# Leqr/MSMP-PDE

Measured on AMD Instinct MI355X. Metric: rollout-steps/sec (whole node), E2 nx=100 tw=25, higher is better.
Workload: dtype f32; 1 GPU; E2 MSMP-PDE (MP_PDE_SolverLEMLinGated), 2048 graphs x nx=100, time_window=25, 6 gated layer pairs, radius graph n=3; graphs_total=2048, graphs_per_gpu=2048, nodes_per_gpu=204800, edges_per_gpu=1204224, parallelism=dp1 (graph-sharded, no collective in the rollout), sub_batches=1, range_policy_switched_to_exact_fp32=False, preheat=163 untimed steps (>= 1 s) after the 5 warm-up steps

## Files before the change

### msmp-pde_amd/csrc/mlp_kernels.hip

```cpp
#include "mfma_tiles.h"

namespace msmp {

struct EdgeArgs {
    const float* h;
    const float* u;
    const float* pos;
    const float* vars;
    const int* tgt;
    const int* col;
    const int* rowptr;
    long n_edges, n_nodes;
    int tile_nodes;
    int xcd_map;
    int tw, nv, nc1;
    const float* w1;
    const float* w2;
    const float* w2s;
    const float* scales;
    const float* b1;
    const float* b2;
    const float* P;
    const float* Q;
    float* msg;
// ... 730 lines not shown
        const f32x4 v0 = *reinterpret_cast<const f32x4*>(row32 + 16 * s + 8 * hh);
        const f32x4 v1 = *reinterpret_cast<const f32x4*>(row32 + 16 * s + 8 * hh + 4);
        const float v[8] = {v0[0], v0[1], v0[2], v0[3], v1[0], v1[1], v1[2], v1[3]};
        split8(v, bhi[0][s], blo[0][s]);
    }
}

struct NodeSplitArgs {
    NodeArgs b;
    const float* w3s;
    const float* scales;
};

__device__ __forceinline__ void node_head_split(const float* __restrict__ h, const float* __restrict__ agg, const float* __restrict__ vars,
                                                long nc, int nv, const float* b3, const float* b4, const float* w3v, const float* w3s,
                                                const float* scales, float* lds, int tid, int lane, int hh, f32x16 (&y)[4][1]) {
    const float sc3 = scales[2], inv3 = scales[6], sc4 = scales[3], inv4 = scales[7];
    f32x16 z[4][1];
    acc_init_bias<1>(b3, hh, z);
    for (int v = 0; v < nv; ++v) {
        const float xv = vars[(size_t)nc * nv + v];
#pragma unroll
        for (int T = 0; T < 4; ++T)
#pragma unroll
            for (int r = 0; r < 16; ++r)
                z[T][0][r] = fmaf(w3v[(32 * T + acc_row(r, hh)) * MSMP_MAX_VARS + v], xv, z[T][0][r]);
    }
#pragma unroll
    for (int T = 0; T < 4; ++T)
#pragma unroll
        for (int r = 0; r < 16; ++r) z[T][0][r] *= sc3;

    f32x4 pf[4][4];
    auto row_load = [&](int ch, f32x4 (&dst)[4]) {
        const float* row32 = (ch < 4 ? h : agg) + (size_t)nc * H + 32 * (ch & 3);
#pragma unroll
        for (int s = 0; s < 2; ++s) {
            dst[2 * s] = *reinterpret_cast<const f32x4*>(row32 + 16 * s + 8 * hh);
            dst[2 * s + 1] = *reinterpret_cast<const f32x4*>(row32 + 16 * s + 8 * hh + 4);
        }
    };
#pragma unroll
    for (int ch = 0; ch < 4; ++ch) row_load(ch, pf[ch]);
    WStage ws;
    wstage_load(ws, w3s, tid);
    wstage_store_linear(ws, lds, tid);
    __syncthreads();
#pragma unroll
    for (int ch = 0; ch < 8; ++ch) {
        wstage_load(ws, w3s + (size_t)(ch + 1) * SPLIT_CHUNK_FLOATS, tid);
        half8 bhi[1][2], blo[1][2];
#pragma unroll
        for (int s = 0; s < 2; ++s) {
            const f32x4 v0 = pf[ch & 3][2 * s], v1 = pf[ch & 3][2 * s + 1];
            const float v[8] = {v0[0], v0[1], v0[2], v0[3], v1[0], v1[1], v1[2], v1[3]};
            split8(v, bhi[0][s], blo[0][s]);
        }
        if (ch + 4 < 8) row_load(ch + 4, pf[ch & 3]);
        mma_chunk_split<1>(lds + (ch & 1) * SPLIT_CHUNK_FLOATS, lane, bhi, blo, z);
        wstage_store_linear(ws, lds + ((ch + 1) & 1) * SPLIT_CHUNK_FLOATS, tid);
        __syncthreads();
    }
#pragma unroll
    for (int T = 0; T < 4; ++T)
#pragma unroll
        for (int r = 0; r < 16; ++r) z[T][0][r] = swishf(z[T][0][r] * inv3);

    acc_init_bias_scaled<1>(b4, sc4, hh, y);
    const float* w4s = w3s + 8 * SPLIT_CHUNK_FLOATS;
#pragma unroll
    for (int t = 0; t < 4; ++t) {
        if (t < 3) wstage_load(ws, w4s + (size_t)(t + 1) * SPLIT_CHUNK_FLOATS, tid);
        half8 bhi[1][2], blo[1][2];
        split_acc_tile<1>(z[t], bhi, blo);
        mma_chunk_split<1>(lds + (t & 1) * SPLIT_CHUNK_FLOATS, lane, bhi, blo, y);
        if (t < 3) {
            wstage_store_linear(ws, lds + ((t + 1) & 1) * SPLIT_CHUNK_FLOATS, tid);
            __syncthreads();
        }
    }
#pragma unroll
    for (int T = 0; T < 4; ++T)
#pragma unroll
        for (int r = 0; r < 16; ++r) y[T][0][r] *= inv4;
}

__global__ __launch_bounds__(256, 2) void node_update_split_kernel(NodeSplitArgs sa) {
    __shared__ __attribute__((aligned(16))) float lds[2 * SPLIT_CHUNK_FLOATS];
    const NodeArgs& a = sa.b;
    const int tid = threadIdx.x, lane = tid & 63, wave = tid >> 6;
    const int c = lane & 31, hh = lane >> 5;
    const long n = (long)blockIdx.x * 128 + wave * 32 + c;
    const long nc = n < a.n_nodes ? n : a.n_nodes - 1;
    f32x16 y[4][1];
    node_head_split(a.h, a.agg, a.vars, nc, a.nv, a.b3, a.b4, a.w3v, sa.w3s, sa.scales, lds, tid, lane, hh, y);
    if (n < a.n_nodes) {
        float* o = a.out + (size_t)n * H + 4 * hh;
        const float* hx = a.h + (size_t)n * H + 4 * hh;
#pragma unroll
        for (int T = 0; T < 4; ++T)
#pragma unroll
            for (int q = 0; q < 4; ++q) {
                f32x4 v;
                if (a.mode == MSMP_LAYER_LIN) {
#pragma unroll
                    for (int m = 0; m < 4; ++m) v[m] = y[T][0][4 * q + m];
                } else {
                    const f32x4 x = *reinterpret_cast<const f32x4*>(hx + 32 * T + 8 * q);
#pragma unroll
                    for (int m = 0; m < 4; ++m) v[m] = x[m] + swishf(y[T][0][4 * q + m]);
                }
                *reinterpret_cast<f32x4*>(o + 32 * T + 8 * q) = v;
            }
    }
}

struct TailArgs {
    const float* h;
    const float* agg[2];
    const float* vars;
    const int* graph_ptr;
    int nv, mode;
    float eps;
    const float* b3[2];
    const float* b4[2];
    const float* w3vh[2];
    const float* w3s[2];
    const float* w4t[2];
    const float* scales[2];
    float* out;
    int* status;
};

constexpr float TAIL_ACT_SCALE = 64.0f;
constexpr float TAIL_NODE_SCALE = 256.0f;
__device__ __forceinline__ float tail_node_scaled(float x) { return __builtin_amdgcn_fmed3f(x * TAIL_NODE_SCALE, -65504.0f, 65504.0f); }

constexpr int ROWBUF_FLOATS = 128 * 32;
__device__ __forceinline__ void tail_rows_issue(const float* __restrict__ h, const float* __restrict__ agg, int n0, int n1, int ch, float* buf, int tid) {
    const float* src = (ch < 4 ? h : agg) + 32 * (ch & 3);
#pragma unroll
    for (int i = 0; i < 4; ++i) {
        const int P = tid + 256 * i, r = P >> 3;
        const int node = min(n0 + r, n1 - 1);
        const float* g = src + (size_t)node * H + 4 * ((P & 7) ^ ((r >> 1) & 7));
        __builtin_amdgcn_global_load_lds((const __attribute__((address_space(1))) void*)g, (__attribute__((address_space(3))) void*)(buf + 4 * P), 16, 0, 0);
    }
}
__device__ __forceinline__ void tail_rows_read(const float* buf, int row, int hh, f32x4 (&dst)[4]) {
    const float* rb = buf + row * 32;
    const int sw = (row >> 1) & 7;
#pragma unroll
    for (int s = 0; s < 2; ++s) {
        dst[2 * s] = *reinterpret_cast<const f32x4*>(rb + 4 * ((4 * s + 2 * hh) ^ sw));
        dst[2 * s + 1] = *reinterpret_cast<const f32x4*>(rb + 4 * ((4 * s + 2 * hh + 1) ^ sw));
    }
}

__device__ __forceinline__ void wstage_dma(const float* __restrict__ chunk, float* buf, int tid) {
#pragma unroll
    for (int i = 0; i < 4; ++i)
        __builtin_amdgcn_global_load_lds((const __attribute__((address_space(1))) void*)(chunk + 4 * (tid + 256 * i)),
                                         (__attribute__((address_space(3))) void*)(buf + 4 * (tid + 256 * i)), 16, 0, 0);
}

__device__ __forceinline__ void tail_bias_load(const float* b3, int hh, f32x16 (&z)[4][1]) {
#pragma unroll
    for (int T = 0; T < 4; ++T)
#pragma unroll
        for (int q = 0; q < 4; ++q) {
            const f32x4 bv = *reinterpret_cast<const f32x4*>(b3 + 32 * T + 8 * q + 4 * hh);
#pragma unroll
            for (int m = 0; m < 4; ++m) z[T][0][4 * q + m] = bv[m];
        }
}
__device__ __forceinline__ void tail_bias_pin(f32x16 (&z)[4][1]) {
#pragma unroll
    for (int T = 0; T < 4; ++T) asm volatile("" : "+v"(z[T][0]));
}
__device__ __forceinline__ void tail_bias_scale(f32x16 (&z)[4][1], float sc3) {
#pragma unroll
    for (int T = 0; T < 4; ++T)
#pragma unroll
        for (int r = 0; r < 16; ++r) z[T][0][r] *= sc3;
}
__device__ __forceinline__ float tail_sc3(const float* scales) { return uniform_ro(scales, 2) * TAIL_NODE_SCALE; }

__device__ __forceinline__ void tail_chunk_frags(const float* buf, int myrow, int hh, half8 (&bhi)[1][2], half8 (&blo)[1][2]) {
    f32x4 pf[4];
    tail_rows_read(buf, myrow, hh, pf);
#pragma unroll
    for (int s = 0; s < 2; ++s) {
        const f32x4 v0 = pf[2 * s], v1 = pf[2 * s + 1];
        const float v[8] = {v0[0], v0[1], v0[2], v0[3], v1[0], v1[1], v1[2], v1[3]};
        split8_node(v, bhi[0][s], blo[0][s]);
    }
}

template <int CH0, int PB>
__device__ __forceinline__ void head_chunks(float* rowbuf, int n0, int n1, const float* __restrict__ h, const float* __restrict__ agg, const float* w3vh,
                                            const float* w3s, const float* w4t, float* lds, int tid, int lane, int myrow, int hh, f32x16 (&z)[4][1],
                                            half8 (&wvf)[2][4] PROF_ARGS) {
#pragma unroll
    for (int ch = CH0; ch < 8; ++ch) {
        if (ch < 7) tail_rows_issue(h, agg, n0, n1, ch + 1, rowbuf + ((ch + 1) & 1) * ROWBUF_FLOATS, tid);
        wstage_dma(ch < 7 ? w3s + (size_t)(ch + 1) * SPLIT_CHUNK_FLOATS : w4t, lds + ((ch + 1) & 1) * SPLIT_CHUNK_FLOATS, tid);
        half8 bhi[1][2], blo[1][2];
        tail_chunk_frags(rowbuf + (ch & 1) * ROWBUF_FLOATS, myrow, hh, bhi, blo);
        if (ch == 5) {
            const half8* wv = reinterpret_cast<const half8*>(w3vh) + lane;
#pragma unroll
            for (int m = 0; m < 2; ++m)
#pragma unroll
                for (int T = 0; T < 4; ++T) wvf[m][T] = wv[(m * 4 + T) * 64];
        }
        PROF_MARK(PB);
        mma_chunk_split<1>(lds + (ch & 1) * SPLIT_CHUNK_FLOATS, lane, bhi, blo, z);
        PROF_MARK(PB + 1);
        __syncthreads();
        PROF_MARK(PB + 2);
    }
}

__device__ __forceinline__ void tail_var_frags(const float* xvl, int myrow, int hh, half8 (&bx)[2]) {
    const f32x4 x0 = *reinterpret_cast<const f32x4*>(xvl + 8 * myrow), x1 = *reinterpret_cast<const f32x4*>(xvl + 8 * myrow + 4);
    const float xr[8] = {x0[0], x0[1], x0[2], x0[3], x1[0], x1[1], x1[2], x1[3]};
    float xv[8];
#pragma unroll
    for (int f = 0; f < 8; ++f) xv[f] = tail_node_scaled(xr[f]);
    var_slot_frags(xv, hh, bx);
}

template <typename MidHook, typename LastHook>
__device__ __forceinline__ void head_finish(const float* b4, const float* w4t, const float* scales, float* lds, int tid, int lane, int c, int hh,
                                            f32x16 (&z)[4][1], const half8 (&wvf)[2][4], const half8 (&bx)[2], f32x16 (&yT)[4], MidHook mid_hook,
                                            LastHook last_hook, bool center, float* zref) {
    const float inv3 = uniform_ro(scales, 6) * (TAIL_ACT_SCALE / TAIL_NODE_SCALE), sc4 = uniform_ro(scales, 3) * TAIL_ACT_SCALE;
#pragma unroll
    for (int m = 0; m < 2; ++m)
#pragma unroll
        for (int T = 0; T < 4; ++T) z[T][0] = __builtin_amdgcn_mfma_f32_32x32x16_f16(wvf[m][T], bx[m], z[T][0], 0, 0, 0);
    mid_hook();
    __builtin_amdgcn_sched_barrier(0);
#pragma unroll
    for (int T = 0; T < 4; ++T)
#pragma unroll
        for (int r = 0; r < 16; ++r) {
#if MSMP_PRECISE_ACT
            z[T][0][r] = TAIL_ACT_SCALE * swishf(z[T][0][r] * inv3 * (1.0f / TAIL_ACT_SCALE));
#else
            const float xs = z[T][0][r] * inv3;
            const float e = __builtin_amdgcn_exp2f(xs * (-1.44269504088896340736f / TAIL_ACT_SCALE));
            z[T][0][r] = xs * __builtin_amdgcn_rcpf(1.0f + e);
#endif
        }

    if (center) {
        if ((tid >> 6) == 0 && c == 0) {
#pragma unroll
            for (int T = 0; T < 4; ++T)
#pragma unroll
                for (int q = 0; q < 4; ++q)
                    *reinterpret_cast<f32x4*>(zref + 32 * T + 8 * q + 4 * hh) = f32x4{z[T][0][4 * q], z[T][0][4 * q + 1], z[T][0][4 * q + 2], z[T][0][4 * q + 3]};
        }
        __syncthreads();
#pragma unroll
        for (int T = 0; T < 4; ++T)
#pragma unroll
            for (int q = 0; q < 4; ++q) {
                const f32x4 rv = *reinterpret_cast<const f32x4*>(zref + 32 * T + 8 * q + 4 * hh);
#pragma unroll
                for (int m = 0; m < 4; ++m) z[T][0][4 * q + m] -= rv[m];
            }
    }
    {
        const f32x4 bv = center ? f32x4{0.f, 0.f, 0.f, 0.f} : *reinterpret_cast<const f32x4*>(b4 + 4 * c) * sc4;
#pragma unroll
        for (int T = 0; T < 4; ++T)
#pragma unroll
            for (int r = 0; r < 16; ++r) yT[T][r] = bv[T];
    }
#pragma unroll
    for (int t = 0; t < 4; ++t) {
        if (t < 3) wstage_dma(w4t + (size_t)(t + 1) * SPLIT_CHUNK_FLOATS, lds + ((t + 1) & 1) * SPLIT_CHUNK_FLOATS, tid);
        else last_hook();
        __builtin_amdgcn_sched_barrier(0);
        half8 zhi[1][2], zlo[1][2];
        split_acc_tile<1>(z[t], zhi, zlo);
        const half8* w = reinterpret_cast<const half8*>(lds + (t & 1) * SPLIT_CHUNK_FLOATS) + lane;
#pragma unroll
        for (int s = 0; s < 2; ++s)
#pragma unroll
            for (int T = 0; T < 4; ++T) {
                const half8 whi = w[((s * 4 + T) * 2 + 0) * 64], wlo = w[((s * 4 + T) * 2 + 1) * 64];
                MSMP_MFMA_LOLO(1, yT[T], zlo[0][s], wlo);
                yT[T] = __builtin_amdgcn_mfma_f32_32x32x16_f16(zhi[0][s], wlo, yT[T], 0, 0, 0);
                yT[T] = __builtin_amdgcn_mfma_f32_32x32x16_f16(zlo[0][s], whi, yT[T], 0, 0, 0);
                yT[T] = __builtin_amdgcn_mfma_f32_32x32x16_f16(zhi[0][s], whi, yT[T], 0, 0, 0);
            }
        if (t < 3) __syncthreads();
    }
}

__device__ __forceinline__ void tile_t_total(const float (&v)[4], float* part, float* tot, int tid, int wave, int c, int hh,
                                             float (&out)[4]) {
#pragma unroll
    for (int T = 0; T < 4; ++T) part[(wave * 2 + hh) * H + 32 * T + c] = v[T];
    __syncthreads();
    if (tid < H) {
        float s = 0.f;
#pragma unroll
        for (int p = 0; p < 8; ++p) s += part[p * H + tid];
        tot[tid] = s;
    }
    __syncthreads();
#pragma unroll
    for (int T = 0; T < 4; ++T) out[T] = tot[32 * T + c];
}

__device__ __forceinline__ void tile_t_instance_norm(f32x16 (&x)[4], int wave, int cnt, float unit, float eps, float* part, float* tot,
                                                     int tid, int c, int hh, int* status) {
    const float inv = 1.0f / (float)max(cnt, 1);
    const bool ragged = wave * 32 + 32 > cnt;
    if (ragged) {
#pragma unroll
        for (int T = 0; T < 4; ++T)
#pragma unroll
            for (int r = 0; r < 16; ++r) x[T][r] = wave * 32 + acc_row(r, hh) < cnt ? x[T][r] : 0.f;
    }
    float s[4], m[4];
#pragma unroll
    for (int T = 0; T < 4; ++T) {
        float a0 = 0.f, a1 = 0.f;
#pragma unroll
        for (int r = 0; r < 16; r += 2) { a0 += x[T][r]; a1 += x[T][r + 1]; }
        s[T] = a0 + a1;
    }
    tile_t_total(s, part, tot, tid, wave, c, hh, m);
#pragma unroll
    for (int T = 0; T < 4; ++T) {
        const float mean = m[T] * inv;
        float a0 = 0.f, a1 = 0.f;
#pragma unroll
        for (int r = 0; r < 16; r += 2) {
            x[T][r] -= mean;
            x[T][r + 1] -= mean;
            if (ragged) {
                x[T][r] = wave * 32 + acc_row(r, hh) < cnt ? x[T][r] : 0.f;
                x[T][r + 1] = wave * 32 + acc_row(r + 1, hh) < cnt ? x[T][r + 1] : 0.f;
            }
            a0 = fmaf(x[T][r], x[T][r], a0);
            a1 = fmaf(x[T][r + 1], x[T][r + 1], a1);
        }
        s[T] = a0 + a1;
    }
    tile_t_total(s, part, tot, tid, wave, c, hh, m);
    if (wave == 0 && !(m[0] + m[1] + m[2] + m[3] < 3.0e38f)) status_raise(status, MSMP_STATUS_NONFINITE);
#pragma unroll
    for (int T = 0; T < 4; ++T) {
        const float f = unit * msmp_rsq(m[T] * inv * unit * unit + eps);
#pragma unroll
        for (int r = 0; r < 16; ++r) x[T][r] *= f;
    }
}

template <bool GATED>
__global__ __launch_bounds__(256, 2) void node_tail_split_kernel(TailArgs a) {
    __shared__ __attribute__((aligned(16))) float smem[2 * SPLIT_CHUNK_FLOATS + 2 * ROWBUF_FLOATS + 9 * H + 8 * 128];
    float* const lds = smem;
    float* const rowbuf = smem + 2 * SPLIT_CHUNK_FLOATS;
    float* const part = rowbuf + 2 * ROWBUF_FLOATS;
    float* const tot = part + 8 * H;
    float* const xvl = tot + H;
    const int tid = threadIdx.x, lane = tid & 63, wave = tid >> 6;
    const int c = lane & 31, hh = lane >> 5;
    const int n0 = a.graph_ptr[blockIdx.x], n1 = a.graph_ptr[blockIdx.x + 1];
    const int cnt = n1 - n0;
    if (cnt <= 0) return;

    PROF_DECL
#pragma unroll
    for (int i = 0; i < 4; ++i) {
        const int e = tid + 256 * i, row = e >> 3, f = e & 7;
        const float v = a.vars[(size_t)min(n0 + row, n1 - 1) * a.nv + min(f, a.nv - 1)];
        xvl[e] = v * (row < cnt && f < a.nv ? 1.0f : 0.f);
    }
    const int myrow = wave * 32 + c;
    f32x16 tau[4], y[4];
    f32x16 z[4][1];
    half8 wvf[2][4], bx[2];
    if (GATED) {
        f32x16 zg[4][1];
        tail_rows_issue(a.h, a.agg[1], n0, n1, 0, rowbuf, tid);
        wstage_dma(a.w3s[1], lds, tid);
        tail_bias_load(a.b3[1], hh, zg);
        tail_bias_load(a.b3[0], hh, z);
        tail_bias_pin(zg);
        tail_bias_pin(z);
        tail_bias_scale(zg, tail_sc3(a.scales[1]));
        tail_bias_scale(z, tail_sc3(a.scales[0]));
        __syncthreads();
        PROF_MARK(5);
        half8 bhi[1][2], blo[1][2];
#pragma unroll
        for (int s = 0; s < 8; ++s) {
            const int ch = s >> 1;
            if (!(s & 1)) {
                tail_rows_issue(a.h, a.agg[1], n0, n1, ch + 1, rowbuf + ((ch + 1) & 1) * ROWBUF_FLOATS, tid);
                wstage_dma(a.w3s[0] + (size_t)ch * SPLIT_CHUNK_FLOATS, lds + SPLIT_CHUNK_FLOATS, tid);
                __builtin_amdgcn_sched_barrier(0);
                tail_chunk_frags(rowbuf + (ch & 1) * ROWBUF_FLOATS, myrow, hh, bhi, blo);
                PROF_MARK(6);
                mma_chunk_split<1>(lds, lane, bhi, blo, zg);
            } else {
                wstage_dma(a.w3s[1] + (size_t)(ch + 1) * SPLIT_CHUNK_FLOATS, lds, tid);
                __builtin_amdgcn_sched_barrier(0);
                PROF_MARK(6);
                mma_chunk_split<1>(lds + SPLIT_CHUNK_FLOATS, lane, bhi, blo, z);
            }
            PROF_MARK(7);
            __syncthreads();
            PROF_MARK(8);
        }
        head_chunks<4, 9>(rowbuf, n0, n1, a.h, a.agg[1], a.w3vh[1], a.w3s[1], a.w4t[1], lds, tid, lane, myrow, hh, zg, wvf PROF_PASS);
        tail_var_frags(xvl, myrow, hh, bx);
        head_finish(a.b4[1], a.w4t[1], a.scales[1], lds, tid, lane, c, hh, zg, wvf, bx, tau,
                    [&] { tail_rows_issue(a.h, a.agg[0], n0, n1, 4, rowbuf, tid); },
                    [&] { wstage_dma(a.w3s[0] + (size_t)4 * SPLIT_CHUNK_FLOATS, lds, tid); }, true, tot);
        PROF_MARK(0);
        tile_t_instance_norm(tau, wave, cnt, uniform_ro(a.scales[1], 7) * (1.0f / TAIL_ACT_SCALE), a.eps, part, tot, tid, c, hh, a.status);
#pragma unroll
        for (int T = 0; T < 4; ++T)
#pragma unroll
            for (int r = 0; r < 16; ++r) tau[T][r] = sigmoidf_(tau[T][r]);
        __syncthreads();
        PROF_MARK(1);
        head_chunks<4, 12>(rowbuf, n0, n1, a.h, a.agg[0], a.w3vh[0], a.w3s[0], a.w4t[0], lds, tid, lane, myrow, hh, z, wvf PROF_PASS);
    } else {
        tail_rows_issue(a.h, a.agg[0], n0, n1, 0, rowbuf, tid);
        wstage_dma(a.w3s[0], lds, tid);
        tail_bias_load(a.b3[0], hh, z);
        tail_bias_pin(z);
        tail_bias_scale(z, tail_sc3(a.scales[0]));
        __syncthreads();
        PROF_MARK(5);
        head_chunks<0, 12>(rowbuf, n0, n1, a.h, a.agg[0], a.w3vh[0], a.w3s[0], a.w4t[0], lds, tid, lane, myrow, hh, z, wvf PROF_PASS);
        tail_var_frags(xvl, myrow, hh, bx);
    }
    head_finish(a.b4[0], a.w4t[0], a.scales[0], lds, tid, lane, c, hh, z, wvf, bx, y, [] {}, [] {}, GATED || a.mode == MSMP_LAYER_LIN, tot);
    PROF_MARK(2);
    const size_t base = ((size_t)n0 + wave * 32 + 4 * hh) * H + 4 * c;
    const int lim = cnt - wave * 32 - 4 * hh;
    const bool full = wave * 32 + 32 <= cnt;
    const bool need_h = GATED || a.mode != MSMP_LAYER_LIN;
    f32x4 hx[16];
    if (need_h) {
        if (full) {
#pragma unroll
            for (int r = 0; r < 16; ++r) hx[r] = *reinterpret_cast<const f32x4*>(a.h + base + (size_t)((r & 3) + 8 * (r >> 2)) * H);
        } else {
#pragma unroll
            for (int r = 0; r < 16; ++r) {
                const int row = (r & 3) + 8 * (r >> 2);
                hx[r] = row < lim ? *reinterpret_cast<const f32x4*>(a.h + base + (size_t)row * H) : f32x4{0.f, 0.f, 0.f, 0.f};
            }
        }
    }
    float unit = uniform_ro(a.scales[0], 7) * (1.0f / TAIL_ACT_SCALE);
    if (!GATED && a.mode != MSMP_LAYER_LIN) {
#pragma unroll
        for (int T = 0; T < 4; ++T)
#pragma unroll
            for (int r = 0; r < 16; ++r) y[T][r] = hx[r][T] + swishf(y[T][r] * unit);
        unit = 1.0f;
    }
    tile_t_instance_norm(y, wave, cnt, unit, a.eps, part, tot, tid, c, hh, a.status);
    if (need_h) {
        float mx = 0.f;
#pragma unroll
        for (int r = 0; r < 16; ++r) mx = fmaxf(fmaxf(fmaxf(fabsf(hx[r][0]), fabsf(hx[r][1])), fmaxf(fabsf(hx[r][2]), fabsf(hx[r][3]))), mx);
        if (mx > NODE_RANGE) status_raise(a.status, MSMP_STATUS_NODE_SATURATED);
    }
    PROF_MARK(3);
    if (GATED) {
#pragma unroll
        for (int T = 0; T < 4; ++T)
#pragma unroll
            for (int r = 0; r < 16; ++r) y[T][r] = fmaf(tau[T][r], swishf(y[T][r]) - hx[r][T], hx[r][T]);
    }
    if (full) {
#pragma unroll
        for (int r = 0; r < 16; ++r)
            *reinterpret_cast<f32x4*>(a.out + base + (size_t)((r & 3) + 8 * (r >> 2)) * H) = f32x4{y[0][r], y[1][r], y[2][r], y[3][r]};
    } else {
#pragma unroll
        for (int r = 0; r < 16; ++r) {
            const int row = (r & 3) + 8 * (r >> 2);
            if (row < lim) *reinterpret_cast<f32x4*>(a.out + base + (size_t)row * H) = f32x4{y[0][r], y[1][r], y[2][r], y[3][r]};
        }
    }
    PROF_MARK(4);
    PROF_FLUSH
}

}

using namespace msmp;


extern "C" int msmp_edge_mlp_f32(const float* h, const float* u, const float* pos, const float* vars,
                                 const int32_t* tgt, const int32_t* col, int64_t n_nodes, int64_t n_edges,
                                 int tw, int nv, const float* packed, float* msg_out, msmp_stream_t stream) {
    MSMP_REQUIRE(h && u && pos && vars && tgt && col && packed && msg_out, MSMP_ERR_ARG, "msmp_edge_mlp_f32: null pointer");
    MSMP_REQUIRE(n_nodes > 0 && n_edges >= 0 && tw > 0 && nv >= 1 && nv <= MSMP_MAX_VARS, MSMP_ERR_ARG,
                 "msmp_edge_mlp_f32: bad sizes N=%ld E=%ld tw=%d nv=%d", (long)n_nodes, (long)n_edges, tw, nv);
    MSMP_REQUIRE(n_edges < (1L << 31) && n_nodes < (1L << 31), MSMP_ERR_UNSUPPORTED, "msmp_edge_mlp_f32: int32 index range");
    if (n_edges == 0) return MSMP_OK;
    const PackedLayout L = packed_layout(tw, nv);
    EdgeArgs a{h, u, pos, vars, tgt, col, nullptr, (long)n_edges, (long)n_nodes, 0, 0, tw, nv, L.nc1,
               packed + L.w1, packed + L.w2, packed + L.w2s, packed + L.scales, packed + L.b1, packed + L.b2, nullptr, nullptr, msg_out, nullptr, msmp_tune_get("split") ? status_ptr() : nullptr};
    constexpr int NB = 2;
    const unsigned grid = (unsigned)((n_edges + 128 * NB - 1) / (128 * NB));
    timing_begin(MSMP_K_EDGE_MLP, (hipStream_t)stream);
    hipLaunchKernelGGL((edge_mlp_kernel<NB, false, false>), dim3(grid), dim3(256), 0, (hipStream_t)stream, a);
    timing_end(MSMP_K_EDGE_MLP, (hipStream_t)stream);
    return check_launch("edge_mlp_kernel");
}

extern "C" int msmp_node_project_f32(const float* h, const float* u, const float* pos, const float* vars, int64_t n_nodes,
                                     int tw, int nv, const float* packed, float* p_out, float* q_out, msmp_stream_t stream) {
    MSMP_REQUIRE(h && u && pos && vars && packed && p_out && q_out, MSMP_ERR_ARG, "msmp_node_project_f32: null pointer");
    MSMP_REQUIRE(n_nodes > 0 && n_nodes < (1L << 31) && tw > 0 && nv >= 1 && nv <= MSMP_MAX_VARS, MSMP_ERR_ARG,
                 "msmp_node_project_f32: bad sizes");
    const PackedLayout L = packed_layout(tw, nv);
    ProjArgs a{h, u, pos, vars, (long)n_nodes, tw, nv, L.nc1, packed + L.w1, packed + L.b1, p_out, q_out};
    const unsigned grid = (unsigned)((n_nodes + 127) / 128);
    timing_begin(MSMP_K_NODE_PROJ, (hipStream_t)stream);
    if (msmp_tune_get("split")) {
        ProjSplitArgs sa{a, packed + L.w1t, packed + L.scales};
        hipLaunchKernelGGL(node_proj_split_kernel, dim3(grid), dim3(256), 0, (hipStream_t)stream, sa);
    } else
        hipLaunchKernelGGL(node_proj_kernel, dim3(grid), dim3(256), 0, (hipStream_t)stream, a);
    timing_end(MSMP_K_NODE_PROJ, (hipStream_t)stream);
    return check_launch("node_proj_kernel");
}

constexpr int64_t PAIR_MAX_NODES = 65536;

static int edge_aggregate(const float* h, const float* u, const float* pos, const float* vars, const float* P, const float* Q,
                          const int32_t* rowptr, const int32_t* col, const int32_t* tgt, int64_t n_nodes, int64_t n_edges,
                          int max_in_degree, int tw, int nv, const float* packed, float* agg_out, msmp_stream_t stream,
                          const char* who) {
    MSMP_REQUIRE(rowptr && col && tgt && packed && agg_out, MSMP_ERR_ARG, "%s: null pointer", who);
    MSMP_REQUIRE(n_nodes > 0 && n_edges >= 0 && tw > 0 && nv >= 1 && nv <= MSMP_MAX_VARS && max_in_degree >= 0, MSMP_ERR_ARG,
                 "%s: bad sizes", who);
    MSMP_REQUIRE(n_edges < (1L << 31) && n_nodes < (1L << 31), MSMP_ERR_UNSUPPORTED, "%s: int32 index range", who);
    if (n_edges == 0) {
        const hipError_t me = hipMemsetAsync(agg_out, 0, (size_t)n_nodes * H * sizeof(float), (hipStream_t)stream);
        MSMP_REQUIRE(me == hipSuccess, MSMP_ERR_HIP, "%s: memset: %s", who, hipGetErrorString(me));
        return MSMP_OK;
    }
    MSMP_REQUIRE(max_in_degree <= 256, MSMP_ERR_UNSUPPORTED,
                 "%s: max in-degree %d > 256 (use msmp_edge_mlp_f32 + msmp_scatter_mean_f32)", who, max_in_degree);
    const bool split = msmp_tune_get("split") != 0;
    const int edges_per_tile = (P && max_in_degree <= 128 && msmp_tune_get("edge_nb") != 2) ? 128 : 256;
    const PackedLayout L = packed_layout(tw, nv);
    int tile_nodes = max_in_degree > 0 ? edges_per_tile / max_in_degree : edges_per_tile;
    if (tile_nodes > 256) tile_nodes = 256;
    EdgeArgs a{h, u, pos, vars, tgt, col, rowptr, (long)n_edges, (long)n_nodes, tile_nodes, 0, tw, nv, L.nc1,
               packed + L.w1, packed + L.w2, packed + L.w2s, packed + L.scales, packed + L.b1, packed + L.b2, P, Q, nullptr, agg_out, split ? status_ptr() : nullptr};
    const unsigned grid = (unsigned)((n_nodes + tile_nodes - 1) / tile_nodes);
    timing_begin(MSMP_K_EDGE_MLP, (hipStream_t)stream);
    if (P && edges_per_tile == 128 && split) hipLaunchKernelGGL((edge_mlp_kernel_occ2<1, true, true, true>), dim3(grid), dim3(256), 0, (hipStream_t)stream, a);
    else if (P && edges_per_tile == 128) hipLaunchKernelGGL((edge_mlp_kernel<1, true, true>), dim3(grid), dim3(256), 0, (hipStream_t)stream, a);
    else if (P) hipLaunchKernelGGL((edge_mlp_kernel<2, true, true>), dim3(grid), dim3(256), 0, (hipStream_t)stream, a);
    else hipLaunchKernelGGL((edge_mlp_kernel<2, true, false>), dim3(grid), dim3(256), 0, (hipStream_t)stream, a);
    timing_end(MSMP_K_EDGE_MLP, (hipStream_t)stream);
    return check_launch("edge_mlp_kernel<fused mean>");
}

int msmp_pair_project_aggregate(const float* h, const float* u, const float* pos, const float* vars, const int32_t* rowptr,
                                const int32_t* col, const int32_t* tgt, int64_t n_nodes, int64_t n_edges, int max_in_degree, int tw,
                                int nv, const float* packed_a, const float* packed_b, float* p_a, float* q_a, float* p_b, float* q_b,
                                float* agg_a, float* agg_b, msmp_stream_t stream) {
    const int pair = msmp_tune_get("pair");
    if (!pair || (pair == 1 && n_nodes > PAIR_MAX_NODES)) return MSMP_ERR_UNSUPPORTED;
    if (!msmp_tune_get("split") || msmp_tune_get("edge_nb") == 2) return MSMP_ERR_UNSUPPORTED;
    if (n_edges <= 0 || max_in_degree <= 0 || max_in_degree > 128 || n_edges >= (1L << 31) || n_nodes >= (1L << 31)) return MSMP_ERR_UNSUPPORTED;
    const PackedLayout L = packed_layout(tw, nv);
    hipStream_t st = (hipStream_t)stream;
    ProjSplitArgs2 pa;
    const float* packed[2] = {packed_a, packed_b};
    float* pp[2] = {p_a, p_b};
    float* qq[2] = {q_a, q_b};
    float* agg[2] = {agg_a, agg_b};
    for (int i = 0; i < 2; ++i)
        pa.head[i] = ProjSplitArgs{ProjArgs{h, u, pos, vars, (long)n_nodes, tw, nv, L.nc1, packed[i] + L.w1, packed[i] + L.b1, pp[i], qq[i]},
                                   packed[i] + L.w1t, packed[i] + L.scales};
    timing_begin(MSMP_K_NODE_PROJ, st);
    hipLaunchKernelGGL(node_proj_split_pair_kernel, dim3((unsigned)((n_nodes + 127) / 128), 2), dim3(256), 0, st, pa);
    timing_end(MSMP_K_NODE_PROJ, st);
    int tile_nodes = 128 / max_in_degree;
    if (tile_nodes > 256) tile_nodes = 256;
    EdgeArgs2 ea;
    for (int i = 0; i < 2; ++i)
        ea.head[i] = EdgeArgs{nullptr, nullptr, nullptr, nullptr, tgt, col, rowptr, (long)n_edges, (long)n_nodes, tile_nodes, 0, tw, nv, L.nc1,
                              packed[i] + L.w1, packed[i] + L.w2, packed[i] + L.w2s, packed[i] + L.scales, packed[i] + L.b1,
                              packed[i] + L.b2, pp[i], qq[i], nullptr, agg[i], status_ptr()};
    timing_begin(MSMP_K_EDGE_MLP, st);
    hipLaunchKernelGGL(edge_mlp_pair_kernel_occ2, dim3((unsigned)((n_nodes + tile_nodes - 1) / tile_nodes), 2), dim3(256), 0, st, ea);
    timing_end(MSMP_K_EDGE_MLP, st);
    return check_launch("edge_mlp_pair_kernel_occ2");
}

extern "C" int msmp_edge_aggregate_f32(const float* h, const float* u, const float* pos, const float* vars,
                                       const int32_t* rowptr, const int32_t* col, const int32_t* tgt, int64_t n_nodes,
                                       int64_t n_edges, int max_in_degree, int tw, int nv, const float* packed,
                                       float* agg_out, msmp_stream_t stream) {
    MSMP_REQUIRE(h && u && pos && vars, MSMP_ERR_ARG, "msmp_edge_aggregate_f32: null pointer");
    return edge_aggregate(h, u, pos, vars, nullptr, nullptr, rowptr, col, tgt, n_nodes, n_edges, max_in_degree, tw, nv, packed,
                          agg_out, stream, "msmp_edge_aggregate_f32");
}

extern "C" int msmp_edge_aggregate_projected_f32(const float* p, const float* q, const int32_t* rowptr, const int32_t* col,
                                                 const int32_t* tgt, int64_t n_nodes, int64_t n_edges, int max_in_degree,
                                                 int tw, int nv, const float* packed, float* agg_out, msmp_stream_t stream) {
    MSMP_REQUIRE(p && q, MSMP_ERR_ARG, "msmp_edge_aggregate_projected_f32: null pointer");
    return edge_aggregate(nullptr, nullptr, nullptr, nullptr, p, q, rowptr, col, tgt, n_nodes, n_edges, max_in_degree, tw, nv,
                          packed, agg_out, stream, "msmp_edge_aggregate_projected_f32");
}

#if MSMP_PROF
extern "C" __attribute__((visibility("default"))) int msmp_debug_prof(unsigned long long* out16, int reset) {
    if (reset) { unsigned long long z[16] = {0}; return (int)hipMemcpyToSymbol(HIP_SYMBOL(g_prof), z, sizeof(z)); }
    return (int)hipMemcpyFromSymbol(out16, HIP_SYMBOL(g_prof), 16 * sizeof(unsigned long long));
}
#endif

extern "C" int msmp_node_tail_f32(const float* h, const float* agg_main, const float* agg_gate, const float* vars,
                                  const int32_t* graph_ptr, int64_t n_nodes, int64_t n_graphs, int max_graph_nodes, int nv,
                                  const float* packed_main, const float* packed_gate, int mode, float eps, float* out,
                                  msmp_stream_t stream) {
    MSMP_REQUIRE(h && agg_main && vars && graph_ptr && packed_main && out, MSMP_ERR_ARG, "msmp_node_tail_f32: null pointer");
    MSMP_REQUIRE((agg_gate != nullptr) == (packed_gate != nullptr), MSMP_ERR_ARG, "msmp_node_tail_f32: give both gate arguments or none");
    MSMP_REQUIRE(n_nodes > 0 && n_graphs > 0 && n_graphs < (1L << 31) && nv >= 1 && nv <= MSMP_MAX_VARS, MSMP_ERR_ARG,
                 "msmp_node_tail_f32: bad sizes");
    MSMP_REQUIRE(mode == MSMP_LAYER_LIN || mode == MSMP_LAYER_RESIDUAL_SWISH, MSMP_ERR_ARG, "msmp_node_tail_f32: bad mode %d", mode);
    MSMP_REQUIRE(!packed_gate || mode == MSMP_LAYER_LIN, MSMP_ERR_ARG, "msmp_node_tail_f32: the gated pair uses GNN_LayerLin layers");
    MSMP_REQUIRE(out != h, MSMP_ERR_ARG, "msmp_node_tail_f32: out may not alias h");
    MSMP_REQUIRE(max_graph_nodes > 0 && max_graph_nodes <= 128, MSMP_ERR_UNSUPPORTED,
                 "msmp_node_tail_f32: graphs of up to 128 nodes (got max_graph_nodes=%d); use the piecewise entry points", max_graph_nodes);
    MSMP_REQUIRE(msmp_tune_get("split"), MSMP_ERR_UNSUPPORTED, "msmp_node_tail_f32: only on the fp16-split matrix path");
    const PackedLayout L = packed_layout(1, nv);
    const float* pg = packed_gate ? packed_gate : packed_main;
    TailArgs a{h, {agg_main, agg_gate}, vars, graph_ptr, nv, mode, eps,
               {packed_main + L.b3, pg + L.b3}, {packed_main + L.b4, pg + L.b4}, {packed_main + L.w3vh, pg + L.w3vh},
               {packed_main + L.w3s, pg + L.w3s}, {packed_main + L.w4t, pg + L.w4t}, {packed_main + L.scales, pg + L.scales}, out, status_ptr()};
    timing_begin(MSMP_K_NODE_UPDATE, (hipStream_t)stream);
    if (packed_gate) hipLaunchKernelGGL(node_tail_split_kernel<true>, dim3((unsigned)n_graphs), dim3(256), 0, (hipStream_t)stream, a);
    else hipLaunchKernelGGL(node_tail_split_kernel<false>, dim3((unsigned)n_graphs), dim3(256), 0, (hipStream_t)stream, a);
    timing_end(MSMP_K_NODE_UPDATE, (hipStream_t)stream);
    return check_launch("node_tail_split_kernel");
}

extern "C" int msmp_node_update_f32(const float* h, const float* agg, const float* vars, int64_t n_nodes, int nv,
                                    const float* packed, int mode, float* out, msmp_stream_t stream) {
    MSMP_REQUIRE(h && agg && vars && packed && out, MSMP_ERR_ARG, "msmp_node_update_f32: null pointer");
    MSMP_REQUIRE(n_nodes > 0 && nv >= 1 && nv <= MSMP_MAX_VARS, MSMP_ERR_ARG, "msmp_node_update_f32: bad sizes");
    MSMP_REQUIRE(mode == MSMP_LAYER_LIN || mode == MSMP_LAYER_RESIDUAL_SWISH, MSMP_ERR_ARG, "msmp_node_update_f32: bad mode %d", mode);
    MSMP_REQUIRE(out != h, MSMP_ERR_ARG, "msmp_node_update_f32: out may not alias h");
    const PackedLayout L = packed_layout(1, nv);
    NodeArgs a{h, agg, vars, (long)n_nodes, nv, mode, packed + L.w3, packed + L.w4,
               packed + L.b3, packed + L.b4, packed + L.w3v, out};
    constexpr int NB = 1;
    const unsigned grid = (unsigned)((n_nodes + 128 * NB - 1) / (128 * NB));
    timing_begin(MSMP_K_NODE_UPDATE, (hipStream_t)stream);
    if (msmp_tune_get("split")) {
        NodeSplitArgs sa{a, packed + L.w3s, packed + L.scales};
        hipLaunchKernelGGL(node_update_split_kernel, dim3(grid), dim3(256), 0, (hipStream_t)stream, sa);
    } else
        hipLaunchKernelGGL(node_update_kernel<NB>, dim3(grid), dim3(256), 0, (hipStream_t)stream, a);
    timing_end(MSMP_K_NODE_UPDATE, (hipStream_t)stream);
    return check_launch("node_update_kernel");
}
```

Before: 159.1 rollout-steps/s.

## Prefetch gated-blend h rows into LDS during head_finish via async DMA

In the gated tail kernel, the h rows needed for the final gated blend are now loaded with global_load_lds async copies. These are issued from hooks inside head_finish into free LDS buffers (rowbuf, xvl, lds), so the loads overlap the head compute. After instance norm, waves read their rows back from LDS, and only wave 3's upper rows still load directly from global memory. This aims to hide global load latency on the blend path, at the cost of reusing LDS buffers whose lifetimes must not overlap and of more complex row mapping.

```diff
diff --git a/msmp-pde_amd/csrc/mlp_kernels.hip b/msmp-pde_amd/csrc/mlp_kernels.hip
--- a/msmp-pde_amd/csrc/mlp_kernels.hip
+++ b/msmp-pde_amd/csrc/mlp_kernels.hip
@@ -1056,6 +1056,30 @@
     }
 }
 
+constexpr int BLEND_REG_ROW0 = 104;
+constexpr int BLEND_REG_R0 = 4;
+template <int PIECES>
+__device__ __forceinline__ void blend_rows_issue(const float* __restrict__ h, int n0, int n1, int row0, float* buf, int tid) {
+#pragma unroll
+    for (int i = 0; i < PIECES; ++i) {
+        if ((i & 3) == 0 && n0 + row0 + 8 * i >= n1) break;
+        const int P = tid + 256 * i;
+        const int node = min(n0 + row0 + (P >> 5), n1 - 1);
+        const float* g = h + (size_t)node * H + 4 * (P & 31);
+        __builtin_amdgcn_global_load_lds((const __attribute__((address_space(1))) void*)g, (__attribute__((address_space(3))) void*)(buf + 4 * P), 16, 0, 0);
+    }
+}
+template <int NR>
+__device__ __forceinline__ void blend_rows_read(const float* blk, bool live, int c, int hh, f32x4 (&hx)[16]) {
+    if (live) {
+#pragma unroll
+        for (int r = 0; r < NR; ++r) hx[r] = *reinterpret_cast<const f32x4*>(blk + acc_row(r, hh) * H + 4 * c);
+    } else {
+#pragma unroll
+        for (int r = 0; r < NR; ++r) hx[r] = f32x4{0.f, 0.f, 0.f, 0.f};
+    }
+}
+
 __device__ __forceinline__ void tile_t_total(const float (&v)[4], float* part, float* tot, int tid, int wave, int c, int hh,
                                              float (&out)[4]) {
 #pragma unroll
@@ -1201,20 +1225,28 @@
         head_chunks<0, 12>(rowbuf, n0, n1, a.h, a.agg[0], a.w3vh[0], a.w3s[0], a.w4t[0], lds, tid, lane, myrow, hh, z, wvf PROF_PASS);
         tail_var_frags(xvl, myrow, hh, bx);
     }
-    head_finish(a.b4[0], a.w4t[0], a.scales[0], lds, tid, lane, c, hh, z, wvf, bx, y, [] {}, [] {}, GATED || a.mode == MSMP_LAYER_LIN, tot);
+    head_finish(a.b4[0], a.w4t[0], a.scales[0], lds, tid, lane, c, hh, z, wvf, bx, y,
+                [&] {
+                    if (GATED) blend_rows_issue<8>(a.h, n0, n1, 0, rowbuf, tid);
+                    if (GATED) blend_rows_issue<1>(a.h, n0, n1, 96, xvl, tid);
+                },
+                [&] { if (GATED) blend_rows_issue<4>(a.h, n0, n1, 64, lds, tid); },
+                GATED || a.mode == MSMP_LAYER_LIN, tot);
     PROF_MARK(2);
     const size_t base = ((size_t)n0 + wave * 32 + 4 * hh) * H + 4 * c;
     const int lim = cnt - wave * 32 - 4 * hh;
     const bool full = wave * 32 + 32 <= cnt;
     const bool need_h = GATED || a.mode != MSMP_LAYER_LIN;
+    constexpr int R0 = GATED ? BLEND_REG_R0 : 0;
+    const bool reg_h = GATED ? wave == 3 && cnt > BLEND_REG_ROW0 : need_h;
     f32x4 hx[16];
-    if (need_h) {
+    if (reg_h) {
         if (full) {
 #pragma unroll
-            for (int r = 0; r < 16; ++r) hx[r] = *reinterpret_cast<const f32x4*>(a.h + base + (size_t)((r & 3) + 8 * (r >> 2)) * H);
+            for (int r = R0; r < 16; ++r) hx[r] = *reinterpret_cast<const f32x4*>(a.h + base + (size_t)((r & 3) + 8 * (r >> 2)) * H);
         } else {
 #pragma unroll
-            for (int r = 0; r < 16; ++r) {
+            for (int r = R0; r < 16; ++r) {
                 const int row = (r & 3) + 8 * (r >> 2);
                 hx[r] = row < lim ? *reinterpret_cast<const f32x4*>(a.h + base + (size_t)row * H) : f32x4{0.f, 0.f, 0.f, 0.f};
             }
@@ -1229,6 +1261,16 @@
         unit = 1.0f;
     }
     tile_t_instance_norm(y, wave, cnt, unit, a.eps, part, tot, tid, c, hh, a.status);
+    if (GATED) {
+        if (wave < 3) blend_rows_read<16>(wave < 2 ? rowbuf + wave * ROWBUF_FLOATS : lds, wave * 32 < cnt, c, hh, hx);
+        else {
+            blend_rows_read<R0>(xvl, cnt > 96, c, hh, hx);
+            if (!reg_h) {
+#pragma unroll
+                for (int r = R0; r < 16; ++r) hx[r] = f32x4{0.f, 0.f, 0.f, 0.f};
+            }
+        }
+    }
     if (need_h) {
         float mx = 0.f;
 #pragma unroll
```

Result: no change. 159.9 rollout-steps/s (median of 6 runs) (+0.5%).
